# facebookresearch/robust_cvd

Hardware: NVIDIA H100
Metric: flow_residual_constraints_per_sec_per_gn_iteration (higher is better)
Workload: dtype f64

## Files before the change

include/rcvd_hooks.h:

```cpp
#ifndef RCVD_HOOKS_H_
#define RCVD_HOOKS_H_
#include "rcvd.h"
#ifdef __cplusplus
extern "C" {
#endif

int64_t rcvd_launch_count(rcvd_problem* p);
int64_t rcvd_filter_launch_count(void);
int64_t rcvd_builder_launch_count(void);
int64_t rcvd_static_flag_launch_count(void);
int64_t rcvd_tracks_launch_count(void);
int64_t rcvd_builder_last_rounds(void);

int32_t rcvd_structure_info(rcvd_problem* p, int32_t out[8]);

int32_t rcvd_debug_factor_plan(const rcvd_config* cfg, int32_t np, const int32_t* pairs, int32_t nt, const int32_t* trip_centers,
                               int32_t order_slack, int32_t nranks, int32_t rank, int32_t num_sms,
                               int32_t* order, int32_t* level, int32_t* owner, int32_t* perm, int32_t out[13]);
int32_t rcvd_debug_update_passes(const rcvd_config* cfg, int32_t np, const int32_t* pairs, int32_t nt, const int32_t* trip_centers,
                                 int32_t order_slack, int32_t nranks, int32_t rank, int32_t num_sms,
                                 int32_t* passes, int32_t* sources, int32_t* join, int32_t counts[5]);

int32_t rcvd_debug_linear_solve(rcvd_problem* p, const double* S, const double* D2, const double* b, double* y);

int32_t rcvd_debug_solve_matrix(rcvd_problem* p, const double* H, const double* D2, const double* b, double* y);
int32_t rcvd_debug_factor_dense(rcvd_problem* p, int32_t* order, double* L, double* Linv);
int32_t rcvd_debug_linear_paths(rcvd_problem* p, int64_t out[13]);

int32_t rcvd_debug_linear_residual(rcvd_problem* p, double radius, double out[6]);

int32_t rcvd_debug_last_iteration(rcvd_problem* p, double* g, double* xc, double out[2]);

int32_t rcvd_debug_profile_linear(rcvd_problem* p, int32_t reps, double out_ms[8]);
int32_t rcvd_debug_level_profile(rcvd_problem* p, double* out, int32_t max_levels);
int32_t rcvd_debug_fp64_tensor_peak(int32_t device, int32_t shape, double* tflops);

int32_t rcvd_debug_set_fast_path(rcvd_problem* p, int32_t on);
int32_t rcvd_debug_set_overlap(rcvd_problem* p, int32_t on);
int32_t rcvd_debug_set_order_slack(rcvd_problem* p, int32_t slack);
int32_t rcvd_debug_set_eval_only(rcvd_problem* p, int32_t on);
int32_t rcvd_debug_set_distributed(rcvd_problem* p, int32_t on);
int32_t rcvd_distribution_info(rcvd_problem* p, int32_t out[4]);
int32_t rcvd_debug_set_update_kernel(rcvd_problem* p, int32_t tma, int32_t side_items_per_cta);

// ... 5 lines not shown
```

robust_cvd_b200/csrc/rcvd_api.cu:

```cuda
#include <algorithm>
#include <chrono>
#include <cmath>
#include <cstdarg>
#include <cstdio>
#include <cstring>
#include <dlfcn.h>
#include <limits>
#include <string>
#include <vector>

#include <cub/device/device_segmented_sort.cuh>
#include "rcvd_eval.cuh"
#include "rcvd_linalg.cuh"
#include "rcvd_update.cuh"
#include "rcvd_plan.h"
#include "rcvd_host.h"

using namespace rcvd;

static thread_local std::string g_err = "";
int set_err(int code, const char* fmt, ...) {
  char buf[512]; va_list ap; va_start(ap, fmt); vsnprintf(buf, sizeof(buf), fmt, ap); va_end(ap);
  g_err = buf; return code;
}
// ... 136 lines not shown
  HBlock *d_hblocks = nullptr, *d_lblocks = nullptr; int* d_fail = nullptr;
  int* d_potrf_progress = nullptr;
  int trsm2_ctas_per_sm = 0;
  FactorPlan plan;
  int *d_lvl_frames = nullptr; GemmTask* d_trsm_tasks = nullptr; int2 *d_trsm_pairs = nullptr, *d_upd_pairs = nullptr;
  SubTask* d_sub_tasks = nullptr; int* d_sub_counters = nullptr; int* d_sub_need = nullptr;
  SolveTask* d_fwd_tasks = nullptr; TrsmTask* d_trsm_ll = nullptr; bool use_trsm_ll = false;
  cudaGraphExec_t solve_graph = nullptr;
  bool structure_ready = false, constraints_set = false, frames_set = false;
  int nranks = 1, rank = 0; nccl::Comm comm = nullptr;
  int64_t launches = 0, graph_launches = 0;
  std::vector<double> h_state; bool state_dirty = false; bool overlap = true; int order_slack = 4;
  cudaStream_t side_stream = nullptr; cudaEvent_t ev_fork = nullptr, ev_join = nullptr;
  std::vector<cudaEvent_t> ev_side;
  cudaStream_t inv_stream = nullptr; cudaEvent_t ev_inv_join = nullptr;
  double *d_g2 = nullptr, *d_delta = nullptr; int* h_fail = nullptr;
  cudaEvent_t ev[8] = {nullptr};
  std::vector<void*> allocs;
  std::vector<std::pair<int, cudaEvent_t>>* prof = nullptr;
  bool eval_only = false;
  bool records_sorted = false;
  int fast_path = 1;
  bool dist_enabled = true, graph_warm = false, force_full_H = false;
  int *d_lvl_own = nullptr, *d_own_lblocks = nullptr, *d_own_hblocks = nullptr, *d_uperm = nullptr;
  UpdItem* d_upd_items = nullptr; CUtensorMap tmapT; int num_sms = 0, upd_ipc = 0;
  std::vector<double> level_ms;
  bool factored = false;
  int64_t paths[LP_N] = {0}, graph_paths[LP_N] = {0};
  rcvd_problem() {}
};

template <class... Params, class... Args>
static int launch(rcvd_problem* p, void (*kernel)(Params...), dim3 grid, dim3 block, size_t smem, cudaStream_t s, bool pdl, Args... args) {
  cudaLaunchAttribute attr = {};
  attr.id = cudaLaunchAttributeProgrammaticStreamSerialization; attr.val.programmaticStreamSerializationAllowed = 1;
  cudaLaunchConfig_t lc = {};
  lc.gridDim = grid; lc.blockDim = block; lc.dynamicSmemBytes = smem; lc.stream = s; lc.attrs = &attr; lc.numAttrs = pdl ? 1 : 0;
  CK(cudaLaunchKernelEx(&lc, kernel, args...));
  p->launches += 1;
  return RCVD_OK;
}

template <class T> static int dalloc(rcvd_problem* p, T** ptr, size_t count) {
  *ptr = nullptr;
  if (count == 0) count = 1;
  cudaError_t e = cudaMallocAsync((void**)ptr, count * sizeof(T), p->stream);
  if (e != cudaSuccess) return set_err(RCVD_ERR_CUDA, "cudaMallocAsync(%zu bytes) failed: %s", count * sizeof(T), cudaGetErrorString(e));
// ... 31 lines not shown
  const DevProblem d = dev_problem(p);
  const RegCounts rcn = reg_counts(p->cfg, p->L, p->N, p->nscale);
  const int regblocks = (rcn.total + 127) / 128;
  cudaStream_t st = p->stream; double* part = p->d_partial; int rc;
  if (p->num_tiles > 0) {
    const bool tc = MODE == EvalMode::CostGradH && p->fast_path != 0;
    if (tc && p->fast_path == 1 && p->records_sorted) rc = launch(p, k_accumulate_runs, p->num_tiles, kTile, kRunSmem, st, false, d, x, p->d_H, g, part);
    else if (tc && fast_path_ok(p->cfg, p->L)) rc = launch(p, k_accumulate_fast, p->num_tiles, kTile, kFastSmem, st, false, d, x, p->d_H, g, part);
    else rc = launch(p, k_pairs<MODE>, p->num_tiles, kTile, 0, st, false, d, x, p->d_H, g, part, p->d_active);
    if (rc) return rc;
  }
  part += p->num_tiles;
  if (regblocks > 0 && (rc = launch(p, k_regularisers<MODE>, regblocks, 128, 0, st, false, d, rcn, x, p->d_H, g, part, p->d_active, p->first_frame, p->last_frame))) return rc;
  part += regblocks;
  if (p->num_trip_tiles > 0 && (rc = launch(p, k_triplets<MODE>, p->num_trip_tiles, kTile, 0, st, false, d, x, p->d_H, g, part, p->d_active))) return rc;
  return RCVD_OK;
}

#define UP(ptr, vec) if ((rc = upload(p, &(ptr), vec))) return rc
#define DA(ptr, n) if ((rc = dalloc(p, &(ptr), (n)))) return rc
static int upload_plan(rcvd_problem* p) {
  const FactorPlan& pl = p->plan; int rc;
  UP(p->d_blk_of, pl.blk_of); UP(p->d_hblocks, pl.hblocks); UP(p->d_lblocks, pl.lblocks); UP(p->d_lvl_frames, pl.lvl_frames); UP(p->d_lvl_own, pl.lvl_own);
  UP(p->d_own_lblocks, pl.own_lblocks); UP(p->d_own_hblocks, pl.own_hblocks); UP(p->d_uperm, pl.uperm);
  UP(p->d_trsm_tasks, pl.trsm_tasks); UP(p->d_trsm_pairs, pl.trsm_pairs); UP(p->d_upd_pairs, pl.upd_pairs);
  UP(p->d_sub_tasks, pl.sub_tasks); UP(p->d_sub_need, pl.sub_need); DA(p->d_sub_counters, (size_t)4 * p->N + 4);
  UP(p->d_fwd_tasks, pl.fwd_tasks); UP(p->d_trsm_ll, pl.trsm_ll); UP(p->d_upd_items, pl.upd_items);
  return RCVD_OK;
}

static int set_up_problem_data(rcvd_problem* p) {
  const int N = p->N; const Layout& L = p->L; const std::vector<int>& uperm = p->plan.uperm; int rc;
  const int np = (int)(p->pair_frames.size() / 2);
  std::vector<int32_t> tile_pair, tile_count; std::vector<int64_t> tile_begin;
  for (int i = 0; i < np; ++i)
    for (int64_t b = p->offsets[i]; b < p->offsets[i + 1]; b += kTile) { tile_pair.push_back(i); tile_begin.push_back(b); tile_count.push_back((int32_t)std::min<int64_t>(kTile, p->offsets[i + 1] - b)); }
  p->num_tiles = (int)tile_pair.size(); p->C = p->offsets.empty() ? 0 : p->offsets.back();
  UP(p->d_tile_pair, tile_pair); UP(p->d_tile_begin, tile_begin); UP(p->d_tile_count, tile_count);
  {
    std::vector<int32_t> pf_int(p->pair_frames.size());
    for (size_t i = 0; i < pf_int.size(); ++i) pf_int[i] = p->plan.iperm[p->pair_frames[i]];
    UP(p->d_pair_frames, pf_int); UP(p->d_records, p->records_h);
  }
  p->records_sorted = false;
  if (run_path_ok(p->cfg, L) && p->C > 0 && p->C < (int64_t)0x7fffffff) {
    const long long n = p->C;
    unsigned *d_k0 = nullptr, *d_k1 = nullptr; int *d_i0 = nullptr, *d_i1 = nullptr; float* d_sorted = nullptr; int64_t* d_off = nullptr; void* d_tmp = nullptr;
// ... 282 lines not shown
      SubCounters cn; cn.ticket = p->d_sub_counters; cn.fin = p->d_sub_counters + 4; cn.fdone = cn.fin + N; cn.bin = cn.fdone + N; cn.bdone = cn.bin + N;
      cn.fin_need = p->d_sub_need; cn.bin_need = p->d_sub_need + N;
      const int ntasks = (int)pl.sub_tasks.size();
      if ((rc = launch(LP_SUB_FUSED, k_substitution, dim3(std::min(ntasks, p->num_sms)), dim3(kSubThreads), substitution_smem_bytes(npad), st, false,
                       p->d_invL, p->d_T, p->d_rhs, p->d_ytmp, p->d_y, p->d_sub_tasks, ntasks, cn, npad))) return rc;
    }
    for (int l = LS - 1; l >= 0; --l) {
      const Level& lv = pl.levels[l];
      if (lv.nfwd > 0 && (rc = launch(LP_SUB_LEVEL, k_bwd_update, dim3((npad + 31) / 32, lv.nfwd), dim3(256), 0, st, false, p->d_T, p->d_y, p->d_ytmp,
                                      p->d_fwd_tasks + lv.fwd_off, npad))) return rc;
      if ((rc = launch(LP_SUB_LEVEL, k_bwd_diag, dim3((npad + 31) / 32, lv.nframes), dim3(256), 0, st, false, p->d_invL, p->d_ytmp, p->d_y,
                       p->d_lvl_frames + lv.frame_off, npad))) return rc;
    }
    mark(P_SOLVE);
    return RCVD_OK;
  }
};

static int enqueue_factor_solve(rcvd_problem* p) {
  FactorSolve f(p);
  const FactorPlan& pl = p->plan; const int npad = p->L.npad, nlv = (int)pl.levels.size();
  f.mark(-1);
  CK(cudaMemsetAsync(p->d_potrf_progress, 0, (size_t)p->N * sizeof(int), p->stream));
  if (int rc = f.launch(LP_OTHER, k_load_factor, dim3((npad * npad + 255) / 256, pl.dist ? (int)pl.own_lblocks.size() : p->N + pl.nLoff), dim3(256), 0,
                        p->stream, false, p->d_H, p->d_Lb, p->d_lblocks, p->d_S, p->d_D2, npad, p->L.nf, pl.dist ? p->d_own_lblocks : nullptr)) return rc;
  f.mark(FactorSolve::P_LOAD);
  for (int li = 0; li < nlv; ++li) {
    const Level& lv = pl.levels[li]; f.prof_level = li;
    if (pl.dist && li == pl.LB) { if (int rc = f.phase_boundary()) return rc; }
    if (lv.nown > 0) {
      const int* frames = p->d_lvl_own + lv.own_off;
      const bool chain = f.streamed(lv);
      if (int rc = f.factor_diagonal(frames, lv.nown, chain && li > 0)) return rc;
      f.mark(FactorSolve::P_POTRF);
      if (int rc = f.trsm(lv, frames, lv.nown, chain)) return rc;
    }
    if (pl.dist && li < pl.LB) { if (int rc = f.broadcast_level(li)) return rc; }
    if (int rc = f.updates(li)) return rc;
  }
  if (pl.dist && pl.LB >= nlv) { if (int rc = f.phase_boundary()) return rc; }
  if (int rc = f.join_all(nlv)) return rc;
  if (int rc = f.substitution()) return rc;
  CK(cudaGetLastError());
  return RCVD_OK;
}

static int factor_solve(rcvd_problem* p) {
  if (p->nranks > 1 && !p->graph_warm) {
// ... 775 lines not shown
                                       order_slack, nranks, rank, true, num_sms))
    return set_err(RCVD_ERR_INVALID, "%s", e);
  return RCVD_OK;
}
RCVD_API int32_t rcvd_debug_factor_plan(const rcvd_config* cfg, int32_t np, const int32_t* pairs, int32_t nt, const int32_t* trip_centers,
                                        int32_t order_slack, int32_t nranks, int32_t rank, int32_t num_sms,
                                        int32_t* order, int32_t* level, int32_t* owner, int32_t* perm, int32_t out[13]) {
  if (!order || !level || !owner || !perm || !out) return set_err(RCVD_ERR_INVALID, "null or negative argument");
  FactorPlan pl;
  if (int32_t rc = debug_plan(pl, cfg, np, pairs, nt, trip_centers, order_slack, nranks, rank, num_sms)) return rc;
  const int N = cfg->num_frames;
  for (int i = 0; i < N; ++i) {
    const int f = pl.uperm[i];
    order[i] = pl.uperm[pl.elim_order[i]]; level[f] = pl.level[i]; owner[f] = pl.owner[i]; perm[i] = f;
  }
  const int32_t v[13] = {(int32_t)pl.levels.size(), pl.nLoff, (int32_t)pl.hblocks.size(), pl.upd_targets, (int32_t)pl.upd_items.size(), (int32_t)pl.sub_tasks.size(),
                         pl.dist ? 1 : 0, pl.LB, pl.sub_first_level, (int32_t)pl.own_lblocks.size(), (int32_t)pl.own_hblocks.size(),
                         pl.dist ? pl.fa_cnt[rank] + pl.fb_cnt[rank] : N, (int32_t)pl.upd_tasks.size()};
  std::copy(v, v + 13, out);
  return RCVD_OK;
}
RCVD_API int32_t rcvd_debug_update_passes(const rcvd_config* cfg, int32_t np, const int32_t* pairs, int32_t nt, const int32_t* trip_centers,
                                          int32_t order_slack, int32_t nranks, int32_t rank, int32_t num_sms,
                                          int32_t* passes, int32_t* sources, int32_t* join, int32_t counts[5]) {
  if (!counts) return set_err(RCVD_ERR_INVALID, "null argument");
  FactorPlan pl;
  if (int32_t rc = debug_plan(pl, cfg, np, pairs, nt, trip_centers, order_slack, nranks, rank, num_sms)) return rc;
  const int32_t need[3] = {(int32_t)pl.upd_tasks.size(), (int32_t)pl.upd_pairs.size(), 2 * (int32_t)pl.levels.size()};
  if (passes) {
    if (!sources || !join || counts[0] < need[0] || counts[1] < need[1] || counts[2] < need[2]) return set_err(RCVD_ERR_INVALID, "null or short output array");
    const int N = cfg->num_frames;
    for (size_t l = 0; l < pl.levels.size(); ++l) {
      const Level& lv = pl.levels[l];
      join[2 * l] = lv.join[0]; join[2 * l + 1] = lv.join[1];
      for (int q = lv.upd_off; q < lv.upd2_off[1] + lv.nupd2[1]; ++q) {
        const GemmTask& t = pl.upd_tasks[q];
        const HBlock& b = pl.lblocks[t.dst];
        int32_t* o = passes + 5 * (size_t)q;
        o[0] = pl.uperm[b.r]; o[1] = pl.uperm[b.c]; o[2] = (int32_t)l; o[3] = q >= lv.upd2_off[1] ? 2 : q >= lv.upd2_off[0] ? 1 : 0; o[4] = t.count;
        for (int i = 0; i < t.count; ++i) sources[t.first + i] = pl.uperm[pl.lblocks[N + pl.upd_pairs[t.first + i].x].c];
      }
    }
  }
  std::copy(need, need + 3, counts); counts[3] = pl.TB; counts[4] = pl.upd_window;
  return RCVD_OK;
}
RCVD_API int32_t rcvd_structure_info(rcvd_problem* p, int32_t out[8]) {
  if (!p) return set_err(RCVD_ERR_INVALID, "null argument");
  SET_DEVICE(p->device);
  int rc = ensure_ready(p); if (rc) return rc;
  out[0] = p->N; out[1] = p->plan.nLoff; out[2] = (int)p->plan.levels.size(); out[3] = (int)p->plan.hblocks.size(); out[4] = p->L.npad; out[5] = p->L.nf; out[6] = p->num_tiles;
  out[7] = p->plan.upd_targets;
  return RCVD_OK;
}
```

robust_cvd_b200/csrc/rcvd_linalg.cuh:

```cuda
#pragma once
#include "rcvd_device.cuh"

namespace rcvd {

constexpr int kPotrfThreads = 256;

__global__ void __launch_bounds__(kPotrfThreads) k_potrf_panel(double* __restrict__ Lb, double* __restrict__ invT,
                                                                const int* __restrict__ frames, int npad, int jb, int* __restrict__ fail) {
  __shared__ double D[16][17];
  __shared__ double Di[16][17];
  const int frame = frames[blockIdx.x];
  double* A = Lb + (size_t)frame * npad * npad;
  double* iT = invT + (size_t)frame * npad * 16;
  const int tid = threadIdx.x;
  const int j0 = jb * 16;
  {
    const int r = tid >> 4, cc = tid & 15;
    D[r][cc] = (cc <= r) ? A[(size_t)(j0 + r) * npad + j0 + cc] : 0.0;
  }
  __syncthreads();
  if (tid < 32) {
    const int i = tid;
    for (int j = 0; j < 16; ++j) {
      if (i == j) {
// ... 764 lines not shown
        double vi[32];
#pragma unroll
        for (int u = 0; u < 32; ++u) { const int i = ib + 8 * u; vi[u] = i < npad ? __ldcg(vin + i) : 0.0; }
#pragma unroll
        for (int u = 0; u < 32; ++u) { const int i = ib + 8 * u; ax += m[u].x * vi[u]; if (tk.type != 3 || i > j) ay += m[u].y * vi[u]; }
      }
      red[rg * (kSubChunk + 2) + 2 * cl] = ax; red[rg * (kSubChunk + 2) + 2 * cl + 1] = ay;
      __syncthreads();
      if (tid < kSubChunk && c0 + tid < c1) {
        double sum = 0.0;
#pragma unroll
        for (int q = 0; q < 8; ++q) sum += red[q * (kSubChunk + 2) + tid];
        if (tk.type == 3) x[(size_t)tk.k * npad + c0 + tid] = sum; else red_add(y + (size_t)tk.k * npad + c0 + tid, -sum);
      }
    }
    __syncthreads();
    if (tid == 0) red_release_add(tk.type == 0 ? cn.fdone + tk.k : (tk.type == 1 ? cn.fin + tk.r : (tk.type == 2 ? cn.bin + tk.k : cn.bdone + tk.k)), 1);
  }
}
__host__ __device__ inline size_t substitution_smem_bytes(int) { return (size_t)8 * (kSubChunk + 2) * sizeof(double); }

struct HBlock { int lblk; int r; int c; };
__global__ void __launch_bounds__(256) k_load_factor(const double* __restrict__ H, double* __restrict__ Lb, const HBlock* __restrict__ lb,
                                                      const double* __restrict__ S, const double* __restrict__ D2, int npad, int nf, const int* __restrict__ blist) {
  const int bid = blist ? blist[blockIdx.y] : blockIdx.y;
  const HBlock b = lb[bid];
  const int e = blockIdx.x * 256 + threadIdx.x;
  if (e >= npad * npad) return;
  const int i = e / npad, j = e % npad;
  const size_t bs = (size_t)npad * npad;
  double v = 0.0;
  if (b.r == b.c) {
    if (j > i) v = 0.0;
    else if (i >= nf) v = (i == j) ? 1.0 : 0.0;
    else {
      v = H[(size_t)b.lblk * bs + e] * S[(size_t)b.r * npad + i] * S[(size_t)b.c * npad + j];
      if (i == j) v += D2[(size_t)b.r * npad + i];
    }
  } else if (b.lblk >= 0 && i < nf && j < nf) {
    v = H[(size_t)b.lblk * bs + e] * S[(size_t)b.r * npad + i] * S[(size_t)b.c * npad + j];
  }
  Lb[(size_t)bid * bs + e] = v;
}

__global__ void __launch_bounds__(256) k_spmv_sym(const double* __restrict__ H, const HBlock* __restrict__ hb, const double* __restrict__ v,
                                                   double* __restrict__ out, int npad, const int* __restrict__ blist) {
  const int bid = blist ? blist[blockIdx.y] : blockIdx.y;
  const HBlock b = hb[bid];
  const int row = blockIdx.x * 8 + (threadIdx.x >> 5);
  const int lane = threadIdx.x & 31;
  if (row >= npad) return;
  const double* M = H + (size_t)bid * npad * npad + (size_t)row * npad;
  const double* vc = v + (size_t)b.c * npad;
  const double vr = v[(size_t)b.r * npad + row];
  double s = 0.0;
  if (b.r == b.c) {
    for (int q = lane; q <= row; q += 32) {
      const double m = M[q];
      s += m * vc[q];
      if (q < row && m != 0.0) red_add(out + (size_t)b.c * npad + q, m * vr);
    }
  } else {
    for (int q = lane; q < npad; q += 32) {
      const double m = M[q];
      s += m * vc[q];
// ... 9 lines not shown
```

robust_cvd_b200/csrc/rcvd_plan.h:

```cpp
#pragma once
#include <algorithm>
#include <map>
#include <set>
#include <vector>

#include "rcvd_linalg.cuh"
#include "rcvd_update.cuh"

namespace rcvd {

struct Level { int frame_off, nframes; int trsm_off, ntrsm; int upd_off, nupd; int upd2_off[2], nupd2[2]; int fwd_off, nfwd; int it_off, nit, it2_off[2], nit2[2]; int own_off, nown; int join[2]; };

constexpr int kUpdWindow = 2, kUpdWindowMaxNf = 256;

struct FactorPlan {
  std::vector<int> elim_order;
  std::vector<int> level, owner;
  std::vector<Level> levels;
  bool dist = false; int LB = 0;
  std::vector<int> uperm, iperm;
  std::vector<int> fa_off, fa_cnt, fb_off, fb_cnt, tseg, bseg, hseg;
  int nLoff = 0;
  std::vector<HBlock> hblocks, lblocks;
  std::vector<int32_t> blk_of;
  std::vector<int> own_lblocks, own_hblocks;
  std::vector<int> lvl_frames, lvl_own;
  std::vector<GemmTask> trsm_tasks, upd_tasks; std::vector<int2> trsm_pairs, upd_pairs;
  std::vector<TrsmTask> trsm_ll; std::vector<SolveTask> fwd_tasks;
  std::vector<UpdItem> upd_items; int upd_rb = 0, upd_neff = 0;
  int upd_targets = 0;
  int upd_window = 1;
  int TB = 0;
  double upd_flops = 0.0;
  std::vector<SubTask> sub_tasks; std::vector<int> sub_need; int sub_first_level = 0;
};

inline const char* make_factor_plan(FactorPlan& P, const rcvd_config& cfg, const std::vector<int32_t>& pairs, const std::vector<int32_t>& trip_centers,
                                    int order_slack, int nranks, int rank, bool dist_enabled, int num_sms) {
  P = FactorPlan();
  Layout L;
  if (!make_layout(cfg, L) || cfg.num_frames <= 0) return "unsupported transform configuration";
  const int N = cfg.num_frames, npad = L.npad;
  std::vector<std::set<int>> adj(N);
  auto addEdge = [&](int a, int b) { if (a != b) { adj[a].insert(b); adj[b].insert(a); } };
  for (size_t i = 0; i + 1 < pairs.size(); i += 2) {
    const int a = pairs[i], b = pairs[i + 1];
    if (a < 0 || a >= N || b < 0 || b >= N) return "pair frame index out of range";
    addEdge(a, b);
// ... 90 lines not shown
  P.blk_of.assign((size_t)N * N, -1);
  for (int f = 0; f < N; ++f) hblocks.push_back({f, f, f});
  P.hseg.assign((size_t)R * 2, 0);
  for (int q = 0; q < R; ++q) {
    P.hseg[(size_t)q * 2] = (int)hblocks.size();
    for (int a = 0; a < N; ++a) for (int b : orig[a]) if (a < b) {
      const int r = pos[a] > pos[b] ? a : b, c = pos[a] > pos[b] ? b : a;
      if (own[c] != q) continue;
      const int hid = (int)hblocks.size();
      hblocks.push_back({lid[{r, c}], r, c});
      P.blk_of[(size_t)r * N + c] = hid * 2 + 1;
      P.blk_of[(size_t)c * N + r] = hid * 2 + 0;
    }
    P.hseg[(size_t)q * 2 + 1] = (int)hblocks.size() - P.hseg[(size_t)q * 2];
  }
  const int nHblocks = (int)hblocks.size();
  P.lblocks.resize(N + nLoff);
  for (int f = 0; f < N; ++f) P.lblocks[f] = {f, f, f};
  for (auto& kv : lid) P.lblocks[kv.second] = {-1, kv.first.first, kv.first.second};
  for (int h = N; h < nHblocks; ++h) P.lblocks[hblocks[h].lblk].lblk = h;
  P.elim_order = order; P.level = lvl; P.owner = own;
  for (int b = 0; b < N + nLoff; ++b) { const int c = b < N ? b : lcol[b - N]; if (!dist || own[c] == rank) P.own_lblocks.push_back(b); }
  for (int h = 0; h < nHblocks; ++h) if (!dist || own[hblocks[h].c] == rank) P.own_hblocks.push_back(h);
  const int upd_neff = std::min(npad, (L.nf + 7) / 8 * 8);
  const int upd_nt = (upd_neff + kUpdMaxTile - 1) / kUpdMaxTile;
  const int upd_tile = std::min(kUpdMaxTile, upd_neff);
  P.upd_rb = upd_tile; P.upd_neff = upd_neff;
  auto col_of = [&](int target) { return target < N ? target : lcol[target - N]; };
  std::map<int, std::vector<std::pair<int, int2>>> prod;
  for (int l = 0; l < nl; ++l) {
    const bool shared_level = !dist || l >= LB;
    std::set<int> targets;
    for (int k : lf[l]) for (size_t a = 0; a < cs[k].size(); ++a) for (size_t b = 0; b <= a; ++b) {
      const int r = cs[k][a], c = cs[k][b];
      if (!shared_level && own[c] != rank) continue;
      const int target = (r == c) ? r : lid[{r, c}];
      prod[target].push_back({l, make_int2(lid[{r, k}] - N, lid[{c, k}] - N)});
      targets.insert(target);
    }
    P.upd_targets += (int)targets.size();
  }
  const int W = P.upd_window = L.nf <= kUpdWindowMaxNf ? kUpdWindow : 1;
  auto window = [&](int l) { return l < TB ? l / W : nl + l; };
  std::vector<std::vector<std::pair<int, std::vector<int2>>>> late(nl), deferred(nl);
  for (auto& kv : prod) {
    const int Lc = lvl[col_of(kv.first)];
    const auto& v = kv.second;
    for (size_t i = 0, j; i < v.size(); i = j) {
      const bool is_late = v[i].first == Lc - 1;
      for (j = i + 1; j < v.size() && (v[j].first == Lc - 1) == is_late && (is_late || window(v[j].first) == window(v[i].first)); ++j) {}
      auto& pass = (is_late ? late : deferred)[v[j - 1].first];
      pass.push_back({kv.first, {}});
      for (size_t q = i; q < j; ++q) pass.back().second.push_back(v[q].second);
    }
  }
  for (int l = 0; l < nl; ++l) {
    Level lv; lv.frame_off = (int)P.lvl_frames.size(); lv.nframes = (int)lf[l].size(); lv.own_off = (int)P.lvl_own.size();
    lv.trsm_off = (int)P.trsm_tasks.size(); lv.upd_off = (int)P.upd_tasks.size(); lv.fwd_off = (int)P.fwd_tasks.size();
    const bool shared_level = !dist || l >= LB;
    for (int k : lf[l]) {
      P.lvl_frames.push_back(k);
      const bool mine = shared_level || own[k] == rank;
      if (mine) P.lvl_own.push_back(k);
      for (int r : cs[k]) {
        const int id = lid[{r, k}];
        if (mine) {
          P.trsm_tasks.push_back({id - N, (int)P.trsm_pairs.size(), 1, 0});
          P.trsm_pairs.push_back(make_int2(id, k));
          P.trsm_ll.push_back({id - N, id, k});
        }
        P.fwd_tasks.push_back({id - N, r, k});
      }
    }
    lv.nown = (int)P.lvl_own.size() - lv.own_off;
    lv.join[0] = lv.join[1] = nl;
    const bool split = W > 1 && l < TB;
    for (int pass = 0; pass < 3; ++pass) {
      if (pass > 0) lv.upd2_off[pass - 1] = (int)P.upd_tasks.size();
      for (auto& tp : (pass ? deferred : late)[l]) {
        const int Lc = lvl[col_of(tp.first)];
        if (pass > 0 && (!split || Lc == l + 2) != (pass == 1)) continue;
        if (pass > 0) lv.join[pass - 1] = std::min(lv.join[pass - 1], Lc - 1);
        P.upd_tasks.push_back({tp.first, (int)P.upd_pairs.size(), (int)tp.second.size(), tp.first < N ? 1 : 0});
        { const double n = (double)L.nf; P.upd_flops += (double)tp.second.size() * (tp.first < N ? n * n * (n + 1.0) : 2.0 * n * n * n); }
        P.upd_pairs.insert(P.upd_pairs.end(), tp.second.begin(), tp.second.end());
      }
    }
    lv.ntrsm = (int)P.trsm_tasks.size() - lv.trsm_off; lv.nupd = lv.upd2_off[0] - lv.upd_off; lv.nfwd = (int)P.fwd_tasks.size() - lv.fwd_off;
    lv.nupd2[0] = lv.upd2_off[1] - lv.upd2_off[0]; lv.nupd2[1] = (int)P.upd_tasks.size() - lv.upd2_off[1];
    std::vector<UpdItem>& items = P.upd_items;
    for (int pass = 0; pass < 3; ++pass) {
      const int t0 = pass ? lv.upd2_off[pass - 1] : lv.upd_off, tn = pass ? lv.nupd2[pass - 1] : lv.nupd;
      const size_t i0 = items.size();
      for (int q = t0; q < t0 + tn; ++q) {
        const GemmTask& tk = P.upd_tasks[q];
        for (int ti = 0; ti < upd_nt; ++ti) for (int tj = 0; tj < ((tk.lower_only & 1) ? ti + 1 : upd_nt); ++tj) {
          UpdItem it; it.dst = tk.dst; it.first = tk.first; it.count = tk.count; it.m0 = (short)(ti * upd_tile); it.n0 = (short)(tj * upd_tile);
          it.mrows = (short)std::min(upd_tile, upd_neff - ti * upd_tile); it.ncols = (short)std::min(upd_tile, upd_neff - tj * upd_tile);
          it.flags = ((tk.lower_only & 1) && ti == tj) ? 1 : 0;
          items.push_back(it);
        }
      }
      auto cost = [](const UpdItem& a) { return (long)a.count * (a.mrows / 8) * (a.ncols / 8) * ((a.flags & 1) ? 3 : 4); };
      std::stable_sort(items.begin() + i0, items.end(), [&](const UpdItem& a, const UpdItem& b) { return cost(a) > cost(b); });
      if (pass) { lv.it2_off[pass - 1] = (int)i0; lv.nit2[pass - 1] = (int)(items.size() - i0); } else { lv.it_off = (int)i0; lv.nit = (int)(items.size() - i0); }
    }
    P.levels.push_back(lv);
  }
  P.sub_need.assign(2 * (size_t)N, 0);
  {
    const int nch = (npad + kSubChunk - 1) / kSubChunk;
    const int limit = 4 * num_sms;
    int LS = (int)P.levels.size();
    while (LS > 0 && (P.levels[LS - 1].nframes + P.levels[LS - 1].nfwd) * nch <= limit) --LS;
    P.sub_first_level = LS;
    for (size_t l = LS; l < P.levels.size(); ++l) {
      const Level& lv = P.levels[l];
      for (int i = 0; i < lv.nframes; ++i) for (int c = 0; c < nch; ++c) P.sub_tasks.push_back({0, -1, -1, P.lvl_frames[lv.frame_off + i], c});
      for (int q = 0; q < lv.nfwd; ++q) { const SolveTask& t = P.fwd_tasks[lv.fwd_off + q]; for (int c = 0; c < nch; ++c) P.sub_tasks.push_back({1, t.blk, t.r, t.k, c}); P.sub_need[t.r] += nch; P.sub_need[N + t.k] += nch; }
    }
    for (int l = (int)P.levels.size() - 1; l >= LS; --l) {
      const Level& lv = P.levels[l];
      for (int q = 0; q < lv.nfwd; ++q) { const SolveTask& t = P.fwd_tasks[lv.fwd_off + q]; for (int c = 0; c < nch; ++c) P.sub_tasks.push_back({2, t.blk, t.r, t.k, c}); }
      for (int i = 0; i < lv.nframes; ++i) for (int c = 0; c < nch; ++c) P.sub_tasks.push_back({3, -1, -1, P.lvl_frames[lv.frame_off + i], c});
    }
  }
// ... 5 lines not shown
```

robust_cvd_b200/csrc/rcvd_update.cuh:

```cuda
#pragma once
#include <cuda.h>
#include <stdint.h>
#include "rcvd_linalg.cuh"

namespace rcvd {

struct UpdItem {
  int dst;
  int first, count;
  short m0, n0;
  short mrows, ncols;
  int flags;
};

constexpr int kUpdMaxTile = 80;
constexpr int kUpdPartial = 4 * 25 * 32 * 2;
template <int TEAMS> struct UpdShape { static constexpr int stages = TEAMS == 2 ? 8 : 5, threads = TEAMS * 128 + 32, ctas = TEAMS == 2 ? 1 : 2; };
__host__ __device__ inline size_t upd_smem_bytes(int rb, int teams) {
  const int stages = teams == 2 ? 8 : 5;
  return (size_t)stages * 2 * rb * 16 * sizeof(double) + (teams == 2 ? (size_t)kUpdPartial * sizeof(double) : 0) + 2 * stages * sizeof(uint64_t) + 1024;
}

__device__ __forceinline__ uint32_t smem_u32(const void* p) { return (uint32_t)__cvta_generic_to_shared(p); }
__device__ __forceinline__ void mbar_init(uint64_t* bar, int count) { asm volatile("mbarrier.init.shared::cta.b64 [%0], %1;" ::"r"(smem_u32(bar)), "r"(count) : "memory"); }
__device__ __forceinline__ void mbar_expect_tx(uint64_t* bar, uint32_t bytes) {
  asm volatile("mbarrier.arrive.expect_tx.shared::cta.b64 _, [%0], %1;" ::"r"(smem_u32(bar)), "r"(bytes) : "memory");
}
__device__ __forceinline__ void mbar_arrive(uint64_t* bar) { asm volatile("mbarrier.arrive.shared::cta.b64 _, [%0];" ::"r"(smem_u32(bar)) : "memory"); }
__device__ __forceinline__ void mbar_wait(uint64_t* bar, uint32_t parity) {
  asm volatile(
      "{\n"
      ".reg .pred P1;\n"
      "LAB_WAIT:\n"
      "mbarrier.try_wait.parity.shared::cta.b64 P1, [%0], %1;\n"
      "@P1 bra DONE;\n"
      "bra LAB_WAIT;\n"
// ... 25 lines not shown
      double af[NI], bf[NJ];
#pragma unroll
      for (int i = 0; i < NI; ++i) af[i] = *reinterpret_cast<const double*>(As + kc[k4] + i * 1024);
#pragma unroll
      for (int j = 0; j < NJ; ++j) bf[j] = *reinterpret_cast<const double*>(Bs + kc[k4] + j * 1024);
      upd_mma<NI, NJ>(af, bf, acc);
    }
  } else {
#pragma unroll
    for (int k4 = 0; k4 < 4; ++k4) {
      if (k4 < k4n) {
        double af[NI], bf[NJ];
#pragma unroll
        for (int i = 0; i < NI; ++i) af[i] = *reinterpret_cast<const double*>(As + kc[k4] + i * 1024);
#pragma unroll
        for (int j = 0; j < NJ; ++j) bf[j] = *reinterpret_cast<const double*>(Bs + kc[k4] + j * 1024);
        upd_mma<NI, NJ>(af, bf, acc);
      }
    }
  }
}

template <int NI, int NJ>
__device__ __forceinline__ void upd_epilogue(double* __restrict__ C, int npad, const double (&acc)[5][5][2], int t, const double* __restrict__ part) {
  const bool hi = (t & 2) != 0;
#pragma unroll
  for (int i = 0; i < NI; ++i) {
    double2 v[NJ];
#pragma unroll
    for (int j = 0; j < NJ; ++j) v[j] = *reinterpret_cast<const double2*>(C + (size_t)i * 8 * npad + j * 8);
#pragma unroll
    for (int j = 0; j < NJ; ++j) {
      double a0 = acc[i][j][0], a1 = acc[i][j][1];
      if (part) { const double2 q = *reinterpret_cast<const double2*>(part + (size_t)(i * 5 + j) * 64); a0 += q.x; a1 += q.y; }
      const double give = hi ? a0 : a1;
      const double got = __shfl_xor_sync(0xffffffffu, give, 2);
      const double lo = hi ? got : a0, up = hi ? a1 : got;
      v[j].x -= lo; v[j].y -= up;
      *reinterpret_cast<double2*>(C + (size_t)i * 8 * npad + j * 8) = v[j];
    }
  }
}
template <int NI, int NJ>
__device__ __forceinline__ void upd_store_partial(double* __restrict__ part, const double (&acc)[5][5][2]) {
#pragma unroll
  for (int i = 0; i < NI; ++i)
#pragma unroll
    for (int j = 0; j < NJ; ++j) *reinterpret_cast<double2*>(part + (size_t)(i * 5 + j) * 64) = make_double2(acc[i][j][0], acc[i][j][1]);
}
__device__ __forceinline__ void named_bar_sync(int id, int n) { asm volatile("bar.sync %0, %1;" ::"r"(id), "r"(n) : "memory"); }
__device__ __forceinline__ void named_bar_arrive(int id, int n) { asm volatile("bar.arrive %0, %1;" ::"r"(id), "r"(n) : "memory"); }

#define RCVD_UPD_CASES(M) \
// ... 18 lines not shown
    asm volatile("fence.mbarrier_init.release.cluster;" ::: "memory");
    asm volatile("fence.proxy.async.shared::cta;" ::: "memory");
  }
  __syncthreads();
  const int nk = (neff + 15) >> 4;
  const size_t bs = (size_t)npad * npad;
  if (warp == 4 * TEAMS) {
    if (lane != 0 || (dbg & 1)) return;
    int stage = 0; uint32_t phase = 0;
    for (int w = blockIdx.x; w < nitems; w += gridDim.x) {
      const UpdItem it = items[w];
      for (int p = 0; p < it.count; ++p) {
        const int2 pr = pairs[it.first + p];
        const int rowA = pr.x * npad + it.m0, rowB = pr.y * npad + it.n0;
        for (int kk = 0; kk < nk; ++kk) {
          mbar_wait(&empty[stage], phase ^ 1);
          unsigned char* sa = ring + (size_t)stage * stage_bytes;
          mbar_expect_tx(&full[stage], (uint32_t)stage_bytes);
          tma_load_2d(sa, &tmap, &full[stage], kk * 16, rowA);
          tma_load_2d(sa + tile_bytes, &tmap, &full[stage], kk * 16, rowB);
          if (++stage == kUpdStages) { stage = 0; phase ^= 1; }
        }
      }
    }
    return;
  }
  const int team = warp >> 2, tw = warp & 3;
  const int g = lane >> 2, t = lane & 3;
  const int pg = ((g & 3) << 1) | (g >> 2);
  int kc[4];
#pragma unroll
  for (int k4 = 0; k4 < 4; ++k4) kc[k4] = (((2 * k4 + (t >> 1)) ^ pg) << 4) + ((t & 1) << 3);
  const int wr = tw >> 1, wc = tw & 1;
  double* mypart = partial + (size_t)tw * (25 * 64) + lane * 2;
  if (TEAMS == 2 && team == 0) named_bar_arrive(2, 256);
  int stage = 0; uint32_t phase = 0; unsigned sidx = 0;
  for (int w = blockIdx.x; w < nitems; w += gridDim.x) {
    const UpdItem it = items[w];
    const int hm = ((it.mrows >> 3) + 1) >> 1 << 3, hn = ((it.ncols >> 3) + 1) >> 1 << 3;
    const int wm = wr * hm, wn = wc * hn;
    int ni = wr ? (it.mrows - hm) >> 3 : hm >> 3, nj = wc ? (it.ncols - hn) >> 3 : hn >> 3;
    if ((it.flags & 1) && wr == 0 && wc == 1) ni = 0;
    if (ni == 0 || nj == 0) { ni = 0; nj = 0; }
    double acc[5][5][2];
#pragma unroll
    for (int i = 0; i < 5; ++i)
#pragma unroll
      for (int j = 0; j < 5; ++j) { acc[i][j][0] = 0.0; acc[i][j][1] = 0.0; }
    const int code = ni * 8 + nj;
    const int steps = it.count * nk;
    int kk = 0;
    for (int s = 0; s < steps; ++s, ++sidx) {
      if (TEAMS == 1 || (int)(sidx & 1u) == team) {
        if (!(dbg & 1)) mbar_wait(&full[stage], phase);
        const int k4n = min(4, (neff - kk * 16 + 3) >> 2);
        const unsigned char* sa = ring + (size_t)stage * stage_bytes + (size_t)(wm + pg) * 128;
        const unsigned char* sb = ring + (size_t)stage * stage_bytes + tile_bytes + (size_t)(wn + pg) * 128;
        switch (code) {
#define RCVD_UPD_STAGE(NI_, NJ_) case NI_ * 8 + NJ_: upd_stage<NI_, NJ_>(sa, sb, kc, k4n, acc); break;
          RCVD_UPD_CASES(RCVD_UPD_STAGE)
#undef RCVD_UPD_STAGE
          default: break;
        }
        __syncwarp();
        if (lane == 0 && !(dbg & 1)) mbar_arrive(&empty[stage]);
      }
      if (++stage == kUpdStages) { stage = 0; phase ^= 1; }
      if (++kk == nk) kk = 0;
    }
    if (TEAMS == 2 && team == 1) {
      named_bar_sync(2, 256);
      switch (code) {
#define RCVD_UPD_PART(NI_, NJ_) case NI_ * 8 + NJ_: upd_store_partial<NI_, NJ_>(mypart, acc); break;
        RCVD_UPD_CASES(RCVD_UPD_PART)
#undef RCVD_UPD_PART
        default: break;
      }
      named_bar_arrive(1, 256);
      continue;
    }
    if (TEAMS == 2) named_bar_sync(1, 256);
    if (dbg & 2) { if (acc[0][0][0] == 1.2345e300) dst[0] = acc[4][4][1] + acc[2][3][0]; if (TEAMS == 2) named_bar_arrive(2, 256); continue; }
    double* C = dst + (size_t)it.dst * bs + (size_t)(it.m0 + wm + pg) * npad + it.n0 + wn + ((t & 1) << 2) + (t & 2);
    switch (code) {
#define RCVD_UPD_EPI(NI_, NJ_) case NI_ * 8 + NJ_: upd_epilogue<NI_, NJ_>(C, npad, acc, t, TEAMS == 2 ? mypart : nullptr); break;
      RCVD_UPD_CASES(RCVD_UPD_EPI)
#undef RCVD_UPD_EPI
      default: break;
    }
    if (TEAMS == 2) named_bar_arrive(2, 256);
  }
}

}
```

robust_cvd_b200/solver.py:

```python
import ctypes as C
import os
import numpy as np

from . import abi

_HERE = os.path.dirname(os.path.abspath(__file__))
_LIB = None


def lib():
    global _LIB
    if _LIB is None:
        path = os.path.join(_HERE, "librcvd_b200.so")
        if not os.path.exists(path):
            raise RuntimeError(f"{path} is missing: run `python -c 'import __graft_entry__ as g; g.build()'` "
                               "(the CUDA extension is mandatory, there is no CPU fallback)")
        L = C.CDLL(path)
        L.rcvd_last_error.restype = C.c_char_p
        L.rcvd_launch_count.restype = C.c_int64
        L.rcvd_problem_create.argtypes = [C.POINTER(abi.Config), C.c_int32, C.POINTER(C.c_void_p)]
        L.rcvd_problem_destroy.argtypes = [C.c_void_p]
        for name in ("rcvd_frame_stride", "rcvd_depth_param_offset", "rcvd_spatial_param_offset"):
            getattr(L, name).argtypes = [C.POINTER(abi.Config)]
        _LIB = L
# ... 24 lines not shown
FACTOR_PLAN_COUNTS = ("levels", "offdiag_factor_blocks", "h_blocks", "update_targets", "update_items", "substitution_tasks",
                      "distributed", "first_replicated_level", "first_substitution_level", "rank_l_blocks", "rank_h_blocks", "rank_frames",
                      "update_passes")


def factor_plan(cfg, pairs, trip_centers=(), order_slack=4, nranks=1, rank=0, num_sms=132):
    n = cfg.num_frames
    pf = np.ascontiguousarray(np.asarray(pairs, np.int32).reshape(-1, 2))
    tc = np.ascontiguousarray(np.asarray(trip_centers, np.int32).reshape(-1))
    arrays = {k: np.zeros(n, np.int32) for k in ("order", "level", "owner", "perm")}
    out = (C.c_int32 * len(FACTOR_PLAN_COUNTS))()
    _check(lib().rcvd_debug_factor_plan(C.byref(cfg), C.c_int32(pf.shape[0]), _p(pf, C.c_int32), C.c_int32(tc.size), _p(tc, C.c_int32),
                                        C.c_int32(order_slack), C.c_int32(nranks), C.c_int32(rank), C.c_int32(num_sms),
                                        *(_p(a, C.c_int32) for a in arrays.values()), out))
    return {**arrays, **dict(zip(FACTOR_PLAN_COUNTS, list(out)))}


def update_passes(cfg, pairs, trip_centers=(), order_slack=4, nranks=1, rank=0, num_sms=132):
    pf = np.ascontiguousarray(np.asarray(pairs, np.int32).reshape(-1, 2))
    tc = np.ascontiguousarray(np.asarray(trip_centers, np.int32).reshape(-1))
    args = (C.byref(cfg), C.c_int32(pf.shape[0]), _p(pf, C.c_int32), C.c_int32(tc.size), _p(tc, C.c_int32),
            C.c_int32(order_slack), C.c_int32(nranks), C.c_int32(rank), C.c_int32(num_sms))
    counts = (C.c_int32 * 5)()
    _check(lib().rcvd_debug_update_passes(*args, None, None, None, counts))
    passes, sources, join = np.zeros((counts[0], 5), np.int32), np.zeros(counts[1], np.int32), np.zeros(counts[2], np.int32)
    _check(lib().rcvd_debug_update_passes(*args, _p(passes, C.c_int32), _p(sources, C.c_int32), _p(join, C.c_int32), counts))
    return {"passes": passes, "sources": sources, "join": join.reshape(-1, 2), "tail": counts[3], "window": counts[4]}


class Problem:
    def __init__(self, cfg, device=0):
        self.cfg = cfg
        self.L = lib()
        self.h = C.c_void_p()
        _check(self.L.rcvd_problem_create(C.byref(cfg), C.c_int32(device), C.byref(self.h)))
        self.N = cfg.num_frames
        self.stride = frame_stride(cfg)
        self.U = self.N * self.stride
        self.num_constraints = 0

    def close(self):
        if getattr(self, "h", None):
            self.L.rcvd_problem_destroy(self.h)
            self.h = None

    def __del__(self):
        try:
            self.close()
        except Exception:
            pass
# ... 310 lines not shown
```

Baseline: 80.84 million.

## Skip loading zero fill-in blocks; first update writes fresh and only zeroes padding

Fill-in L blocks with no H source are no longer fully zeroed by the load kernel. Only their padding region beyond neff is cleared, and the first Schur update into such a block stores its result directly instead of reading C. This removes a full block write plus a read of zeros from the factorisation. An L2 bulk prefetch of the destination tile is also added in the single-team producer path. Correctness depends on the first-fill detection matching the actual execution order of the update passes.

```diff
diff --git a/include/rcvd_hooks.h b/include/rcvd_hooks.h
--- a/include/rcvd_hooks.h
+++ b/include/rcvd_hooks.h
@@ -19,7 +19,7 @@
                                int32_t* order, int32_t* level, int32_t* owner, int32_t* perm, int32_t out[13]);
 int32_t rcvd_debug_update_passes(const rcvd_config* cfg, int32_t np, const int32_t* pairs, int32_t nt, const int32_t* trip_centers,
                                  int32_t order_slack, int32_t nranks, int32_t rank, int32_t num_sms,
-                                 int32_t* passes, int32_t* sources, int32_t* join, int32_t counts[5]);
+                                 int32_t* passes, int32_t* sources, int32_t* join, int32_t* flags, int32_t counts[5]);
 
 int32_t rcvd_debug_linear_solve(rcvd_problem* p, const double* S, const double* D2, const double* b, double* y);
 
diff --git a/robust_cvd_b200/csrc/rcvd_api.cu b/robust_cvd_b200/csrc/rcvd_api.cu
--- a/robust_cvd_b200/csrc/rcvd_api.cu
+++ b/robust_cvd_b200/csrc/rcvd_api.cu
@@ -182,7 +182,7 @@
   bool records_sorted = false;
   int fast_path = 1;
   bool dist_enabled = true, graph_warm = false, force_full_H = false;
-  int *d_lvl_own = nullptr, *d_own_lblocks = nullptr, *d_own_hblocks = nullptr, *d_uperm = nullptr;
+  int *d_lvl_own = nullptr, *d_load_lblocks = nullptr, *d_own_hblocks = nullptr, *d_uperm = nullptr;
   UpdItem* d_upd_items = nullptr; CUtensorMap tmapT; int num_sms = 0, upd_ipc = 0;
   std::vector<double> level_ms;
   bool factored = false;
@@ -260,7 +260,7 @@
 static int upload_plan(rcvd_problem* p) {
   const FactorPlan& pl = p->plan; int rc;
   UP(p->d_blk_of, pl.blk_of); UP(p->d_hblocks, pl.hblocks); UP(p->d_lblocks, pl.lblocks); UP(p->d_lvl_frames, pl.lvl_frames); UP(p->d_lvl_own, pl.lvl_own);
-  UP(p->d_own_lblocks, pl.own_lblocks); UP(p->d_own_hblocks, pl.own_hblocks); UP(p->d_uperm, pl.uperm);
+  UP(p->d_load_lblocks, pl.load_lblocks); UP(p->d_own_hblocks, pl.own_hblocks); UP(p->d_uperm, pl.uperm);
   UP(p->d_trsm_tasks, pl.trsm_tasks); UP(p->d_trsm_pairs, pl.trsm_pairs); UP(p->d_upd_pairs, pl.upd_pairs);
   UP(p->d_sub_tasks, pl.sub_tasks); UP(p->d_sub_need, pl.sub_need); DA(p->d_sub_counters, (size_t)4 * p->N + 4);
   UP(p->d_fwd_tasks, pl.fwd_tasks); UP(p->d_trsm_ll, pl.trsm_ll); UP(p->d_upd_items, pl.upd_items);
@@ -589,8 +589,9 @@
   const FactorPlan& pl = p->plan; const int npad = p->L.npad, nlv = (int)pl.levels.size();
   f.mark(-1);
   CK(cudaMemsetAsync(p->d_potrf_progress, 0, (size_t)p->N * sizeof(int), p->stream));
-  if (int rc = f.launch(LP_OTHER, k_load_factor, dim3((npad * npad + 255) / 256, pl.dist ? (int)pl.own_lblocks.size() : p->N + pl.nLoff), dim3(256), 0,
-                        p->stream, false, p->d_H, p->d_Lb, p->d_lblocks, p->d_S, p->d_D2, npad, p->L.nf, pl.dist ? p->d_own_lblocks : nullptr)) return rc;
+  const int nfill = (int)pl.load_lblocks.size() - pl.nload;
+  if (int rc = f.launch(LP_OTHER, k_load_factor, dim3((npad * npad + 255) / 256, pl.nload + load_factor_pad_rows(npad, pl.upd_neff, nfill)), dim3(256), 0,
+                        p->stream, false, p->d_H, p->d_Lb, p->d_lblocks, p->d_S, p->d_D2, npad, p->L.nf, pl.upd_neff, p->d_load_lblocks, pl.nload, nfill)) return rc;
   f.mark(FactorSolve::P_LOAD);
   for (int li = 0; li < nlv; ++li) {
     const Level& lv = pl.levels[li]; f.prof_level = li;
@@ -1412,13 +1413,13 @@
 }
 RCVD_API int32_t rcvd_debug_update_passes(const rcvd_config* cfg, int32_t np, const int32_t* pairs, int32_t nt, const int32_t* trip_centers,
                                           int32_t order_slack, int32_t nranks, int32_t rank, int32_t num_sms,
-                                          int32_t* passes, int32_t* sources, int32_t* join, int32_t counts[5]) {
+                                          int32_t* passes, int32_t* sources, int32_t* join, int32_t* flags, int32_t counts[5]) {
   if (!counts) return set_err(RCVD_ERR_INVALID, "null argument");
   FactorPlan pl;
   if (int32_t rc = debug_plan(pl, cfg, np, pairs, nt, trip_centers, order_slack, nranks, rank, num_sms)) return rc;
   const int32_t need[3] = {(int32_t)pl.upd_tasks.size(), (int32_t)pl.upd_pairs.size(), 2 * (int32_t)pl.levels.size()};
   if (passes) {
-    if (!sources || !join || counts[0] < need[0] || counts[1] < need[1] || counts[2] < need[2]) return set_err(RCVD_ERR_INVALID, "null or short output array");
+    if (!sources || !join || !flags || counts[0] < need[0] || counts[1] < need[1] || counts[2] < need[2]) return set_err(RCVD_ERR_INVALID, "null or short output array");
     const int N = cfg->num_frames;
     for (size_t l = 0; l < pl.levels.size(); ++l) {
       const Level& lv = pl.levels[l];
@@ -1428,6 +1429,7 @@
         const HBlock& b = pl.lblocks[t.dst];
         int32_t* o = passes + 5 * (size_t)q;
         o[0] = pl.uperm[b.r]; o[1] = pl.uperm[b.c]; o[2] = (int32_t)l; o[3] = q >= lv.upd2_off[1] ? 2 : q >= lv.upd2_off[0] ? 1 : 0; o[4] = t.count;
+        flags[q] = t.lower_only;
         for (int i = 0; i < t.count; ++i) sources[t.first + i] = pl.uperm[pl.lblocks[N + pl.upd_pairs[t.first + i].x].c];
       }
     }
diff --git a/robust_cvd_b200/csrc/rcvd_linalg.cuh b/robust_cvd_b200/csrc/rcvd_linalg.cuh
--- a/robust_cvd_b200/csrc/rcvd_linalg.cuh
+++ b/robust_cvd_b200/csrc/rcvd_linalg.cuh
@@ -810,13 +810,23 @@
 
 struct HBlock { int lblk; int r; int c; };
 __global__ void __launch_bounds__(256) k_load_factor(const double* __restrict__ H, double* __restrict__ Lb, const HBlock* __restrict__ lb,
-                                                      const double* __restrict__ S, const double* __restrict__ D2, int npad, int nf, const int* __restrict__ blist) {
-  const int bid = blist ? blist[blockIdx.y] : blockIdx.y;
+                                                      const double* __restrict__ S, const double* __restrict__ D2, int npad, int nf, int neff,
+                                                      const int* __restrict__ blist, int nload, int nfill) {
+  const size_t bs = (size_t)npad * npad;
+  if ((int)blockIdx.y >= nload) {
+    const int ph = npad - neff, per = ph * (npad + neff);
+    const long q = ((long)(blockIdx.y - nload) * gridDim.x + blockIdx.x) * 256 + threadIdx.x;
+    if (per == 0 || q >= (long)nfill * per) return;
+    const int f = (int)(q / per), e = (int)(q % per), r = e - ph * npad;
+    const int i = r < 0 ? neff + e / npad : r / ph, j = r < 0 ? e % npad : neff + r % ph;
+    Lb[(size_t)blist[nload + f] * bs + (size_t)i * npad + j] = 0.0;
+    return;
+  }
+  const int bid = blist[blockIdx.y];
   const HBlock b = lb[bid];
   const int e = blockIdx.x * 256 + threadIdx.x;
   if (e >= npad * npad) return;
   const int i = e / npad, j = e % npad;
-  const size_t bs = (size_t)npad * npad;
   double v = 0.0;
   if (b.r == b.c) {
     if (j > i) v = 0.0;
@@ -825,10 +835,14 @@
       v = H[(size_t)b.lblk * bs + e] * S[(size_t)b.r * npad + i] * S[(size_t)b.c * npad + j];
       if (i == j) v += D2[(size_t)b.r * npad + i];
     }
-  } else if (b.lblk >= 0 && i < nf && j < nf) {
+  } else if (i < nf && j < nf) {
     v = H[(size_t)b.lblk * bs + e] * S[(size_t)b.r * npad + i] * S[(size_t)b.c * npad + j];
   }
   Lb[(size_t)bid * bs + e] = v;
+}
+__host__ __device__ inline int load_factor_pad_rows(int npad, int neff, int nfill) {
+  const long per = (long)(npad - neff) * (npad + neff), row = (long)((npad * npad + 255) / 256) * 256;
+  return (int)(((long)nfill * per + row - 1) / row);
 }
 
 __global__ void __launch_bounds__(256) k_spmv_sym(const double* __restrict__ H, const HBlock* __restrict__ hb, const double* __restrict__ v,
diff --git a/robust_cvd_b200/csrc/rcvd_plan.h b/robust_cvd_b200/csrc/rcvd_plan.h
--- a/robust_cvd_b200/csrc/rcvd_plan.h
+++ b/robust_cvd_b200/csrc/rcvd_plan.h
@@ -24,6 +24,7 @@
   std::vector<HBlock> hblocks, lblocks;
   std::vector<int32_t> blk_of;
   std::vector<int> own_lblocks, own_hblocks;
+  std::vector<int> load_lblocks; int nload = 0;
   std::vector<int> lvl_frames, lvl_own;
   std::vector<GemmTask> trsm_tasks, upd_tasks; std::vector<int2> trsm_pairs, upd_pairs;
   std::vector<TrsmTask> trsm_ll; std::vector<SolveTask> fwd_tasks;
@@ -160,19 +161,24 @@
   P.elim_order = order; P.level = lvl; P.owner = own;
   for (int b = 0; b < N + nLoff; ++b) { const int c = b < N ? b : lcol[b - N]; if (!dist || own[c] == rank) P.own_lblocks.push_back(b); }
   for (int h = 0; h < nHblocks; ++h) if (!dist || own[hblocks[h].c] == rank) P.own_hblocks.push_back(h);
+  for (int b : P.own_lblocks) if (P.lblocks[b].lblk >= 0) P.load_lblocks.push_back(b);
+  P.nload = (int)P.load_lblocks.size();
+  for (int b : P.own_lblocks) if (P.lblocks[b].lblk < 0) P.load_lblocks.push_back(b);
   const int upd_neff = std::min(npad, (L.nf + 7) / 8 * 8);
   const int upd_nt = (upd_neff + kUpdMaxTile - 1) / kUpdMaxTile;
   const int upd_tile = std::min(kUpdMaxTile, upd_neff);
   P.upd_rb = upd_tile; P.upd_neff = upd_neff;
   auto col_of = [&](int target) { return target < N ? target : lcol[target - N]; };
   std::map<int, std::vector<std::pair<int, int2>>> prod;
+  std::map<int, int> first_level;
   for (int l = 0; l < nl; ++l) {
     const bool shared_level = !dist || l >= LB;
     std::set<int> targets;
     for (int k : lf[l]) for (size_t a = 0; a < cs[k].size(); ++a) for (size_t b = 0; b <= a; ++b) {
       const int r = cs[k][a], c = cs[k][b];
+      const int target = (r == c) ? r : lid[{r, c}];
+      first_level.emplace(target, l);
       if (!shared_level && own[c] != rank) continue;
-      const int target = (r == c) ? r : lid[{r, c}];
       prod[target].push_back({l, make_int2(lid[{r, k}] - N, lid[{c, k}] - N)});
       targets.insert(target);
     }
@@ -192,6 +198,7 @@
       for (size_t q = i; q < j; ++q) pass.back().second.push_back(v[q].second);
     }
   }
+  std::vector<uint8_t> updated(N + nLoff, 0);
   for (int l = 0; l < nl; ++l) {
     Level lv; lv.frame_off = (int)P.lvl_frames.size(); lv.nframes = (int)lf[l].size(); lv.own_off = (int)P.lvl_own.size();
     lv.trsm_off = (int)P.trsm_tasks.size(); lv.upd_off = (int)P.upd_tasks.size(); lv.fwd_off = (int)P.fwd_tasks.size();
@@ -219,7 +226,9 @@
         const int Lc = lvl[col_of(tp.first)];
         if (pass > 0 && (!split || Lc == l + 2) != (pass == 1)) continue;
         if (pass > 0) lv.join[pass - 1] = std::min(lv.join[pass - 1], Lc - 1);
-        P.upd_tasks.push_back({tp.first, (int)P.upd_pairs.size(), (int)tp.second.size(), tp.first < N ? 1 : 0});
+        const bool first_fill = P.lblocks[tp.first].lblk < 0 && !updated[tp.first] && prod[tp.first][0].first == first_level[tp.first];
+        updated[tp.first] = 1;
+        P.upd_tasks.push_back({tp.first, (int)P.upd_pairs.size(), (int)tp.second.size(), (tp.first < N ? 1 : 0) | (first_fill ? 2 : 0)});
         { const double n = (double)L.nf; P.upd_flops += (double)tp.second.size() * (tp.first < N ? n * n * (n + 1.0) : 2.0 * n * n * n); }
         P.upd_pairs.insert(P.upd_pairs.end(), tp.second.begin(), tp.second.end());
       }
@@ -235,11 +244,11 @@
         for (int ti = 0; ti < upd_nt; ++ti) for (int tj = 0; tj < ((tk.lower_only & 1) ? ti + 1 : upd_nt); ++tj) {
           UpdItem it; it.dst = tk.dst; it.first = tk.first; it.count = tk.count; it.m0 = (short)(ti * upd_tile); it.n0 = (short)(tj * upd_tile);
           it.mrows = (short)std::min(upd_tile, upd_neff - ti * upd_tile); it.ncols = (short)std::min(upd_tile, upd_neff - tj * upd_tile);
-          it.flags = ((tk.lower_only & 1) && ti == tj) ? 1 : 0;
+          it.flags = (((tk.lower_only & 1) && ti == tj) ? kUpdSymDiag : 0) | ((tk.lower_only & 2) ? kUpdFirstFill : 0);
           items.push_back(it);
         }
       }
-      auto cost = [](const UpdItem& a) { return (long)a.count * (a.mrows / 8) * (a.ncols / 8) * ((a.flags & 1) ? 3 : 4); };
+      auto cost = [](const UpdItem& a) { return (long)a.count * (a.mrows / 8) * (a.ncols / 8) * ((a.flags & kUpdSymDiag) ? 3 : 4); };
       std::stable_sort(items.begin() + i0, items.end(), [&](const UpdItem& a, const UpdItem& b) { return cost(a) > cost(b); });
       if (pass) { lv.it2_off[pass - 1] = (int)i0; lv.nit2[pass - 1] = (int)(items.size() - i0); } else { lv.it_off = (int)i0; lv.nit = (int)(items.size() - i0); }
     }
diff --git a/robust_cvd_b200/csrc/rcvd_update.cuh b/robust_cvd_b200/csrc/rcvd_update.cuh
--- a/robust_cvd_b200/csrc/rcvd_update.cuh
+++ b/robust_cvd_b200/csrc/rcvd_update.cuh
@@ -12,6 +12,8 @@
   short mrows, ncols;
   int flags;
 };
+constexpr int kUpdSymDiag = 1;
+constexpr int kUpdFirstFill = 2;
 
 constexpr int kUpdMaxTile = 80;
 constexpr int kUpdPartial = 4 * 25 * 32 * 2;
@@ -83,13 +85,13 @@
 }
 
 template <int NI, int NJ>
-__device__ __forceinline__ void upd_epilogue(double* __restrict__ C, int npad, const double (&acc)[5][5][2], int t, const double* __restrict__ part) {
+__device__ __forceinline__ void upd_epilogue(double* __restrict__ C, int npad, const double (&acc)[5][5][2], int t, const double* __restrict__ part, bool fresh) {
   const bool hi = (t & 2) != 0;
 #pragma unroll
   for (int i = 0; i < NI; ++i) {
     double2 v[NJ];
 #pragma unroll
-    for (int j = 0; j < NJ; ++j) v[j] = *reinterpret_cast<const double2*>(C + (size_t)i * 8 * npad + j * 8);
+    for (int j = 0; j < NJ; ++j) v[j] = fresh ? make_double2(0.0, 0.0) : *reinterpret_cast<const double2*>(C + (size_t)i * 8 * npad + j * 8);
 #pragma unroll
     for (int j = 0; j < NJ; ++j) {
       double a0 = acc[i][j][0], a1 = acc[i][j][1];
@@ -154,6 +156,14 @@
           if (++stage == kUpdStages) { stage = 0; phase ^= 1; }
         }
       }
+      if (TEAMS == 1 && !(it.flags & kUpdFirstFill)) {
+        const int hm = ((it.mrows >> 3) + 1) >> 1 << 3, hn = ((it.ncols >> 3) + 1) >> 1 << 3;
+        const double* row = dst + (size_t)it.dst * bs + (size_t)it.m0 * npad + it.n0;
+        for (int r = 0; r < it.mrows; ++r, row += npad) {
+          const int bytes = ((it.flags & kUpdSymDiag) && r < hm ? hn : it.ncols) * 8;
+          asm volatile("cp.async.bulk.prefetch.L2.global [%0], %1;" ::"l"(row), "r"(bytes) : "memory");
+        }
+      }
     }
     return;
   }
@@ -172,7 +182,7 @@
     const int hm = ((it.mrows >> 3) + 1) >> 1 << 3, hn = ((it.ncols >> 3) + 1) >> 1 << 3;
     const int wm = wr * hm, wn = wc * hn;
     int ni = wr ? (it.mrows - hm) >> 3 : hm >> 3, nj = wc ? (it.ncols - hn) >> 3 : hn >> 3;
-    if ((it.flags & 1) && wr == 0 && wc == 1) ni = 0;
+    if ((it.flags & kUpdSymDiag) && wr == 0 && wc == 1) ni = 0;
     if (ni == 0 || nj == 0) { ni = 0; nj = 0; }
     double acc[5][5][2];
 #pragma unroll
@@ -214,8 +224,9 @@
     if (TEAMS == 2) named_bar_sync(1, 256);
     if (dbg & 2) { if (acc[0][0][0] == 1.2345e300) dst[0] = acc[4][4][1] + acc[2][3][0]; if (TEAMS == 2) named_bar_arrive(2, 256); continue; }
     double* C = dst + (size_t)it.dst * bs + (size_t)(it.m0 + wm + pg) * npad + it.n0 + wn + ((t & 1) << 2) + (t & 2);
+    const bool fresh = (it.flags & kUpdFirstFill) != 0;
     switch (code) {
-#define RCVD_UPD_EPI(NI_, NJ_) case NI_ * 8 + NJ_: upd_epilogue<NI_, NJ_>(C, npad, acc, t, TEAMS == 2 ? mypart : nullptr); break;
+#define RCVD_UPD_EPI(NI_, NJ_) case NI_ * 8 + NJ_: upd_epilogue<NI_, NJ_>(C, npad, acc, t, TEAMS == 2 ? mypart : nullptr, fresh); break;
       RCVD_UPD_CASES(RCVD_UPD_EPI)
 #undef RCVD_UPD_EPI
       default: break;
diff --git a/robust_cvd_b200/solver.py b/robust_cvd_b200/solver.py
--- a/robust_cvd_b200/solver.py
+++ b/robust_cvd_b200/solver.py
@@ -70,10 +70,11 @@
     args = (C.byref(cfg), C.c_int32(pf.shape[0]), _p(pf, C.c_int32), C.c_int32(tc.size), _p(tc, C.c_int32),
             C.c_int32(order_slack), C.c_int32(nranks), C.c_int32(rank), C.c_int32(num_sms))
     counts = (C.c_int32 * 5)()
-    _check(lib().rcvd_debug_update_passes(*args, None, None, None, counts))
+    _check(lib().rcvd_debug_update_passes(*args, None, None, None, None, counts))
     passes, sources, join = np.zeros((counts[0], 5), np.int32), np.zeros(counts[1], np.int32), np.zeros(counts[2], np.int32)
-    _check(lib().rcvd_debug_update_passes(*args, _p(passes, C.c_int32), _p(sources, C.c_int32), _p(join, C.c_int32), counts))
-    return {"passes": passes, "sources": sources, "join": join.reshape(-1, 2), "tail": counts[3], "window": counts[4]}
+    flags = np.zeros(counts[0], np.int32)
+    _check(lib().rcvd_debug_update_passes(*args, _p(passes, C.c_int32), _p(sources, C.c_int32), _p(join, C.c_int32), _p(flags, C.c_int32), counts))
+    return {"passes": passes, "sources": sources, "join": join.reshape(-1, 2), "flags": flags, "tail": counts[3], "window": counts[4]}
 
 
 class Problem:
```

Result: faster. 85.40 million, median of 6 (+5.6%).
